# apschera2023uzk/MWR_fast_forward_operators_and_LBLs

Measured on AMD Instinct MI355X. Metric: TB evaluations/sec (profile x channel x angle), higher is better.
Workload: dtype f64

## Files before the change

### mwr_fast_forward_operators_and_lbls_amd/csrc/mwrt_kernels.hip.h

```cpp
#pragma once
#include <hip/hip_runtime.h>
#include <stdint.h>
#include "../../include/mwrt.h"
#include "mwrt_plan.h"

namespace mwrt {

constexpr double TAUMAX = 125.0;
constexpr double TRANS_MIN = 5.1664206328378610e-55;

struct O2Rec { double f, s300rf2, be, w300, y0, y1, g0, g1, dnu0, dnu1, pad[6]; };
struct H2ORec { double fl, s1, b2, w0, x, w0s, xs, sh, xh, shs, xhs, aair, aself, w2, pad[2]; };
struct ModelFlat : mwrt_model_desc {
  double o2_rf2[MWRT_MAX_O2_LINES];
  O2Rec o2r[MWRT_MAX_O2_LINES];
  H2ORec h2or[MWRT_MAX_H2O_LINES];
};
typedef const __attribute__((address_space(4))) ModelFlat* cmodel;
typedef const __attribute__((address_space(4))) double* cdoubles;

__device__ __forceinline__ int div_small(int n, int d, unsigned magic) {
  return d == 1 ? n : (int)__umulhi((unsigned)n, magic);
}

#ifndef MWRT_EXACT_DIV
#define MWRT_EXACT_DIV 0
#endif
#ifndef MWRT_ABLATE
#define MWRT_ABLATE 0
#endif
#ifndef MWRT_PHASE_CLOCK
#define MWRT_PHASE_CLOCK 0
#endif
#ifndef MWRT_NO_SETPRIO
#define MWRT_NO_SETPRIO 0
#endif
#if MWRT_NO_SETPRIO
#define MWRT_SETPRIO(n) do { } while (0)
#else
#define MWRT_SETPRIO(n) __builtin_amdgcn_s_setprio(n)
#endif
#if MWRT_PHASE_CLOCK
#define MWRT_STAMP(k) do { if (A.phase && lane == 0) A.phase[((int64_t)blockIdx.x * 4 + wave) * 10 + (k)] = (long long)wall_clock64(); } while (0)
#else
#define MWRT_STAMP(k) do { } while (0)
#endif

__device__ __forceinline__ double fdiv(double x, double d) {
#if MWRT_EXACT_DIV
  return x / d;
#else
  double r = __builtin_amdgcn_rcp(d);
  double e = __builtin_fma(-d, r, 1.0);
  r = __builtin_fma(r, e, r);
  e = __builtin_fma(-d, r, 1.0);
  r = __builtin_fma(r, e, r);
  return x * r;
#endif
}

#define MWRT_FMA_SC(p, r, c) asm("v_fma_f64 %0, %1, %2, %3" : "=v"(p) : "v"(p), "v"(r), "s"(c))
__device__ __forceinline__ double fexp(double x) {
#if MWRT_EXACT_DIV
  return exp(x);
#else
  const double k = __builtin_rint(x * 1.4426950408889634074);
  double r = __builtin_fma(k, -6.93147180369123816490e-01, x);
  r = __builtin_fma(k, -1.90821492927058770002e-10, r);
  double p = 2.5100569275813683e-08;
  MWRT_FMA_SC(p, r, 2.762032742826824e-07);
  MWRT_FMA_SC(p, r, 2.75572680728901e-06);
  MWRT_FMA_SC(p, r, 2.4801520792572694e-05);
  MWRT_FMA_SC(p, r, 0.00019841269863303223);
  MWRT_FMA_SC(p, r, 0.0013888888917538296);
  MWRT_FMA_SC(p, r, 0.008333333333330011);
  MWRT_FMA_SC(p, r, 0.04166666666662348);
  MWRT_FMA_SC(p, r, 0.16666666666666669);
  MWRT_FMA_SC(p, r, 0.5000000000000001);
  p = __builtin_fma(p, r, 1.0);
  p = __builtin_fma(p, r, 1.0);
  return __builtin_amdgcn_ldexp(p, (int)k);
#endif
}

__device__ __forceinline__ double two_atanh_tail(double z) {
  double p = 0.14616878919029822;
  MWRT_FMA_SC(p, z, 0.15331686868638428);
  MWRT_FMA_SC(p, z, 0.1818289017031397);
  MWRT_FMA_SC(p, z, 0.22222211120449298);
  MWRT_FMA_SC(p, z, 0.2857142862606338);
  MWRT_FMA_SC(p, z, 0.3999999999989931);
  MWRT_FMA_SC(p, z, 0.666666666666667);
  return p;
}

__device__ __forceinline__ double flog(double x) {
#if MWRT_EXACT_DIV
  return log(x);
#else
  int e = __builtin_amdgcn_frexp_exp(x);
  double m = __builtin_amdgcn_frexp_mant(x);
  const bool lo = m < 0.70710678118654752440;
  m = lo ? m + m : m;
  e = lo ? e - 1 : e;
  const double num = m - 1.0, den = m + 1.0;
  double r = __builtin_amdgcn_rcp(den);
  r = __builtin_fma(r, __builtin_fma(-den, r, 1.0), r);
  r = __builtin_fma(r, __builtin_fma(-den, r, 1.0), r);
  const double s = num * r;
  const double z = s * s;
  const double p = two_atanh_tail(z);
  const double ed = (double)e;
  const double lm = __builtin_fma(s * z, p, s + s);
  return __builtin_fma(ed, 6.93147180369123816490e-01, __builtin_fma(ed, 1.90821492927058770002e-10, lm));
#endif
}

constexpr double EXP_SMALL_X = 0.125;
__device__ __forceinline__ double fexp_small(double x) {
  double p = 2.756514908613403e-06;
  MWRT_FMA_SC(p, x, 2.4810200365624755e-05);
  MWRT_FMA_SC(p, x, 0.00019841269076602318);
  MWRT_FMA_SC(p, x, 0.001388888804772704);
  MWRT_FMA_SC(p, x, 0.008333333333357229);
  MWRT_FMA_SC(p, x, 0.04166666666692954);
  MWRT_FMA_SC(p, x, 0.16666666666666666);
  MWRT_FMA_SC(p, x, 0.4999999999999999);
  p = __builtin_fma(p, x, 1.0);
  return __builtin_fma(p, x, 1.0);
}

__device__ __forceinline__ double ftanh_half_small(double x) {
  const double u = x * x;
  double p = 4.257889640378761e-05;
  MWRT_FMA_SC(p, u, -0.0004216256671577941);
  MWRT_FMA_SC(p, u, 0.004166666662552237);
  MWRT_FMA_SC(p, u, -0.04166666666666466);
  p = __builtin_fma(p, u, 0.5);
  return p * x;
}

constexpr double EXP_TINY_X = 0.015625;
__device__ __forceinline__ double fexp_tiny(double x) {
  double p = 1.3888888888888889e-03;
  MWRT_FMA_SC(p, x, 8.3333333333333332e-03);
  MWRT_FMA_SC(p, x, 4.1666666666666664e-02);
  MWRT_FMA_SC(p, x, 1.6666666666666666e-01);
  p = __builtin_fma(p, x, 0.5);
  p = __builtin_fma(p, x, 1.0);
  return __builtin_fma(p, x, 1.0);
}
__device__ __forceinline__ double ftanh_half_tiny(double x) {
  const double u = x * x;
  double p = -4.2162698412698413e-04;
  MWRT_FMA_SC(p, u, 4.1666666666666666e-03);
  MWRT_FMA_SC(p, u, -4.1666666666666664e-02);
  p = __builtin_fma(p, u, 0.5);
  return p * x;
}

typedef unsigned long long wmask;
__device__ __forceinline__ bool wave_all(bool p) { return __builtin_amdgcn_ballot_w64(!p) == 0ull; }
__device__ __forceinline__ bool wave_any(bool p) { return __builtin_amdgcn_ballot_w64(p) != 0ull; }
__device__ __forceinline__ wmask wballot(bool p) { return __builtin_amdgcn_ballot_w64(p); }
template <class... B>
__device__ __forceinline__ bool wave_all_of(B... b) { return (wballot(b) & ...) == wballot(true); }

__device__ __forceinline__ float row16_max(float m) {
  m = fmaxf(m, __int_as_float(__builtin_amdgcn_update_dpp(0, __float_as_int(m), 0x128, 0xf, 0xf, false)));
  m = fmaxf(m, __int_as_float(__builtin_amdgcn_update_dpp(0, __float_as_int(m), 0x124, 0xf, 0xf, false)));
  m = fmaxf(m, __int_as_float(__builtin_amdgcn_update_dpp(0, __float_as_int(m), 0x122, 0xf, 0xf, false)));
  m = fmaxf(m, __int_as_float(__builtin_amdgcn_update_dpp(0, __float_as_int(m), 0x121, 0xf, 0xf, false)));
  return m;
}
constexpr int K2_SORT_MIN_SEGLEN = 16;

constexpr double PLANCK_SMALL_X = 0.03125;
__device__ __forceinline__ double planck_b(double x, double inv_x) {
  if (wave_all_of(x <= PLANCK_SMALL_X, x > 0.0)) {
    const double u = x * x;
    double g = 3.3068783068783071e-05;
    MWRT_FMA_SC(g, u, -1.3888888888888889e-03);
    MWRT_FMA_SC(g, u, 8.3333333333333329e-02);
    g = __builtin_fma(g, u, 1.0);
    g = __builtin_fma(x, -0.5, g);
    return g * inv_x;
  }
  return fdiv(1.0, fexp(x) - 1.0);
}

__device__ __forceinline__ double fdiv1(double x, double d) {
#if MWRT_EXACT_DIV
  return x / d;
#else
  double r = __builtin_amdgcn_rcp(d);
  r = __builtin_fma(r, __builtin_fma(-d, r, 1.0), r);
  return x * r;
#endif
}

#define LDS_RELOAD_FENCE() asm volatile("" ::: "memory")
#define KEEP_BRANCH() asm volatile("")

typedef const __attribute__((address_space(4))) LineMasks* cmasks;
__device__ __forceinline__ LineMasks load_masks(const LineMasks* table, int chunk) {
  const cmasks q = (cmasks)table + chunk;
  LineMasks lm;
  lm.o2_far = q->o2_far; lm.h2o_far = q->h2o_far; lm.h2o_none = q->h2o_none; lm.h2o_res = q->h2o_res; lm.h2o_sd = q->h2o_sd;
  lm.h2o_sdfar = q->h2o_sdfar; lm.h2o_sdint = q->h2o_sdint;
  lm.h2o_vfar = q->h2o_vfar; lm.o2_vfar = q->o2_vfar; lm.vf_u0 = q->vf_u0; lm.vf_h = q->vf_h; lm.vf_invh = q->vf_invh;
  return lm;
}

struct cplx { double re, im; };
__device__ __forceinline__ cplx cmul(cplx a, cplx b) { return {a.re * b.re - a.im * b.im, a.re * b.im + a.im * b.re}; }
__device__ __forceinline__ cplx cadd(cplx a, double r) { return {a.re + r, a.im}; }
__device__ __forceinline__ cplx crecip(cplx b) {
  const double d = __builtin_fma(b.re, b.re, b.im * b.im);
#if MWRT_EXACT_DIV
  const double r = 1.0 / d;
#else
  double r = __builtin_amdgcn_rcp(d);
  r = __builtin_fma(r, __builtin_fma(-d, r, 1.0), r);
  r = __builtin_fma(r, __builtin_fma(-d, r, 1.0), r);
#endif
  return {b.re * r, -b.im * r};
}
__device__ __forceinline__ cplx cdiv(cplx a, cplx b) { return cmul(a, crecip(b)); }
__device__ __forceinline__ double fsqrt(double x) {
#if MWRT_EXACT_DIV
  return sqrt(x);
#else
  const double y = __builtin_amdgcn_rsq(x);
  double g = x * y;
  const double h = 0.5 * y;
  return __builtin_fma(__builtin_fma(-g, g, x), h, g);
#endif
}
__device__ __forceinline__ cplx csqrt_principal(cplx z) {
  const double r = fsqrt(__builtin_fma(z.re, z.re, z.im * z.im));
  const bool pos = z.re >= 0.0;
  const double a = fsqrt(0.5 * (r + fabs(z.re)));
  const double q = fdiv1(pos ? z.im : fabs(z.im), a + a);
  return pos ? cplx{a, q} : cplx{q, copysign(a, z.im)};
}

__device__ __forceinline__ cplx dcerror_upper(double x, double y) {
  const double a0 = 122.607931777104326, a1 = 214.382388694706425, a2 = 181.928533092181549,
               a3 = 93.155580458138441, a4 = 30.180142196210589, a5 = 5.912626209773153,
               a6 = 0.564189583562615;
  const double b0 = 122.607931773875350, b1 = 352.730625110963558, b2 = 457.334478783897737,
               b3 = 348.703917719495792, b4 = 170.354001821091472, b5 = 53.992906912940207,
               b6 = 10.479857114260399;
  const cplx zh = {fabs(y), -x};
  const double r = zh.re + zh.re;
  const double ms = -__builtin_fma(zh.re, zh.re, zh.im * zh.im);
  auto step = [&](double c, double b1, double b2) -> double { return __builtin_fma(r, b1, __builtin_fma(ms, b2, c)); };
  double n2 = a6, n1 = __builtin_fma(r, a6, a5), nt;
  nt = step(a4, n1, n2); n2 = n1; n1 = nt;
  nt = step(a3, n1, n2); n2 = n1; n1 = nt;
  nt = step(a2, n1, n2); n2 = n1; n1 = nt;
  nt = step(a1, n1, n2); n2 = n1; n1 = nt;
  const cplx as = {__builtin_fma(zh.re, n1, __builtin_fma(ms, n2, a0)), zh.im * n1};
  double d2 = 1.0, d1 = r + b6, dt;
  dt = __builtin_fma(r, d1, ms + b5); d2 = d1; d1 = dt;
  dt = step(b4, d1, d2); d2 = d1; d1 = dt;
  dt = step(b3, d1, d2); d2 = d1; d1 = dt;
  dt = step(b2, d1, d2); d2 = d1; d1 = dt;
  dt = step(b1, d1, d2); d2 = d1; d1 = dt;
  const cplx bs = {__builtin_fma(zh.re, d1, __builtin_fma(ms, d2, b0)), zh.im * d1};
  return cdiv(as, bs);
}

__device__ __forceinline__ double block_sum(double v, double* scratch , int tid, int nthreads) {
#pragma unroll
  for (int o = WAVE / 2; o > 0; o >>= 1) v += __shfl_xor(v, o, WAVE);
  __syncthreads();
  if ((tid & (WAVE - 1)) == 0) scratch[tid / WAVE] = v;
  __syncthreads();
  double s = 0.0;
  for (int w = 0; w < nthreads / WAVE; ++w) s += scratch[w];
  return s;
}

struct LevelState {
  double t;
  double p;
  double rho;
  double pdry;
};

__device__ __forceinline__ double goff_gratch_e(double tk, double rh) {
  const double LN10 = 2.302585092994045684;
  const double INV_LN10 = 0.434294481903251828;
  double y = 373.16 / tk;
  double es = -7.90298 * (y - 1.0) + 5.02808 * (flog(y) * INV_LN10)
            - 1.3816e-07 * (fexp(LN10 * (11.344 * (1.0 - (1.0 / y)))) - 1.0)
            + 0.0081328 * (fexp(LN10 * (-3.49149 * (y - 1.0))) - 1.0) + 3.0057148979490314 ;
  return rh * fexp(LN10 * es);
}

__device__ __forceinline__ LevelState level_state(double p_hpa, double tk, double e) {
  const double rvap = (0.01 * 8.314510) / 18.01528;
  double v = 300.0 / tk;
  double ekpa = e / 10.0;
  double pdrykpa = p_hpa / 10.0 - ekpa;
  LevelState s;
  s.t = 300.0 / v;
  s.p = (pdrykpa + ekpa) * 10.0;
  s.rho = ekpa * 10.0 / (rvap * s.t);
  s.pdry = pdrykpa * 10.0;
  return s;
}

struct H2OLine {
  double c1;
  double w0, wsq;
  double sw;
  double sbase;
  double s;
  double base;
};

__device__ __forceinline__ H2OLine h2o_line(cmodel M, int k, double pda, double pvap, double ti, double tiln,
                                            double ti2, bool shifted) {
  H2OLine q;
  const auto& R = M->h2or[k];
  const double fl = R.fl;
// ... 725 lines not shown
    const double fl = M->x_fl[k];
    const double wc = M->x_w[k] * p * fexp(M->x_x[k] * tiln);
    const double bd = sq * fl;
    const double w = 0.5346 * wc + fsqrt(__builtin_fma(0.2166 * wc, wc, 0.6931 * (bd * bd)));
    const double wsq = w * w;
    const double sw = (M->x_s1[k] * fexp(M->x_b[k] * (1.0 - ti))) * fdiv(w, fl * fl);
    LDS_RELOAD_FENCE();
#pragma unroll
    for (int j = 0; j < NFC; ++j) {
      const double f = sfq[2 * j];
      const double d1 = f - fl, d2 = f + fl;
      const double D1 = __builtin_fma(d1, d1, wsq), D2 = __builtin_fma(d2, d2, wsq);
      const double den12 = D1 * D2;
      double r = __builtin_amdgcn_rcp(den12);
      r = __builtin_fma(r, __builtin_fma(-den12, r, 1.0), r);
      sum[j] = __builtin_fma((D1 + D2) * r, sw, sum[j]);
    }
  }
  const double pref = ((M->x_coef * numden) * qvinv) * fexp(2.5 * tiln);
#pragma unroll
  for (int j = 0; j < NFC; ++j) adry[j] = __builtin_fma(pref * sfq[2 * j + 1], sum[j], adry[j]);
}

#ifdef MWRT_HOST_TU
constexpr double EARTH_RADIUS_KM = 6370.949;
__global__ void __launch_bounds__(1024)
k_ray_paths(const double* __restrict__ z, const double* __restrict__ p, const double* __restrict__ t,
            const double* __restrict__ rh, int nlev, const double* __restrict__ elev_deg, int nang,
            double* __restrict__ amf, uint8_t* __restrict__ duct) {
  __shared__ double seam[16][3];
  const int64_t prof = blockIdx.x;
  const int tid = threadIdx.x, lane = tid & (WAVE - 1), wave = tid / WAVE;
  const bool active = tid < nlev;
  const int64_t off = prof * nlev + (active ? tid : 0);
  const double qnan = __builtin_nan("");
  const double z0 = z[prof * nlev];
  const double zi = z[off] - z0;
  const double pi = p[off], ti = t[off], rhi = rh[off];
  const bool bad_prof = __syncthreads_or(active && (isnan(zi) || isnan(pi) || isnan(ti) || isnan(rhi)));
  const double ni = thayer_refindex(pi, ti, goff_gratch_e(ti, rhi));
  if (lane == WAVE - 1) seam[wave][0] = ni;
  __syncthreads();
  double nprev = __shfl_up(ni, 1, WAVE);
  double zprev = __shfl_up(zi, 1, WAVE);
  if (lane == 0 && wave > 0) { nprev = seam[wave - 1][0]; zprev = z[off - 1] - z0; }
  const double n0 = thayer_refindex(p[prof * nlev], t[prof * nlev], goff_gratch_e(t[prof * nlev], rh[prof * nlev]));
  const double rs = EARTH_RADIUS_KM + 0.0 + z0;
  const double r = EARTH_RADIUS_KM + zi + z0;
  const double rl = EARTH_RADIUS_KM + zprev + z0;
  const double dz = zi - zprev;
  double refbar;
  if (ni == nprev || ni == 1.0 || nprev == 1.0) refbar = (ni + nprev) * 0.5;
  else refbar = 1.0 + (nprev - ni) / (log((nprev - 1.0) / (ni - 1.0)));
  for (int a = 0; a < nang; ++a) {
    double* out = amf + (prof * nang + a) * nlev;
    const double angle = elev_deg[a];
    if (bad_prof || isnan(angle)) {
      if (active) out[tid] = tid == 0 ? 0.0 : qnan;
      continue;
    }
    if ((angle >= 89.0 && angle <= 91.0) || (angle >= -91.0 && angle <= -89.0)) {
      if (active) out[tid] = (tid > 0 && dz != 0.0) ? 1.0 : 0.0;
      continue;
    }
    const double theta0 = angle * (M_PI / 180.0);
    const double costh0 = cos(theta0), sina = sin(theta0 * 0.5);
    const double a0 = 2.0 * (sina * sina);
    const double argdth = zi / rs - ((n0 - ni) * costh0 / ni);
    const double argth = 0.5 * (a0 + argdth) / r;
    const bool trapped_here = active && tid > 0 && !(argth > 0.0);
    double theta = theta0, dtheta = 0.0;
    if (tid > 0 && argth > 0.0) {
      const double sint = sqrt(r * argth);
      theta = 2.0 * asin(sint);
      if ((theta - 2.0 * theta0) <= 0.0) {
        const double dendth = 2.0 * (sint + sina) * cos((theta + theta0) * 0.25);
        const double sind4 = (0.5 * argdth - zi * argth) / dendth;
        dtheta = 4.0 * asin(sind4);
        theta = theta0 + dtheta;
      } else {
        dtheta = theta - theta0;
      }
    }
    const double tanth = tan(theta);
    __syncthreads();
    if (lane == WAVE - 1) { seam[wave][1] = tanth; seam[wave][2] = dtheta; }
    const bool trapped = __syncthreads_or(trapped_here);
    double tanthl = __shfl_up(tanth, 1, WAVE);
    double dthl = __shfl_up(dtheta, 1, WAVE);
    if (lane == 0 && wave > 0) { tanthl = seam[wave - 1][1]; dthl = seam[wave - 1][2]; }
    double f = 0.0;
    if (tid > 0) {
      const double cthbar = ((1.0 / tanth) + (1.0 / tanthl)) * 0.5;
      const double dtau = cthbar * (nprev - ni) / refbar;
      const double dphi = (dtheta - dthl) + dtau;
      const double sh = sin(dphi * 0.5);
      double dsi = sqrt(dz * dz + 4.0 * r * rl * (sh * sh));
      if (dtau != 0.0) {
        const double dtaua = fabs(dtau);
        dsi = dsi * (dtaua / (2.0 * sin(dtaua * 0.5)));
      }
      f = (dz != 0.0) ? dsi / dz : 0.0;
    }
    if (active) out[tid] = trapped ? (tid == 0 ? 0.0 : qnan) : f;
    if (trapped && tid == 0) duct[prof] = 1;
  }
}

#endif

struct FusedArgs {
  const ModelFlat* Ms[MAX_MULTI];
  int64_t nprof_in;
  const double* z; const double* p; const double* t; const double* rh;
  const double* frq;
  const double* airmass;
  double* tb;
  uint8_t* valid;
  double* tbatm; double* tmr; double* tauwet; double* taudry;
  double* taulay;
  int nlev, nf, nang;
  int write_valid;
  LaunchGeom g;
  const double* denliq; const double* denice;
  const double* amf;
  const uint8_t* duct;
  double* tauliq; double* tauice;
  const double* awet_in; const double* adry_in;
  const LineMasks* masks[MAX_MULTI];
  const double* o3n;
#if MWRT_PHASE_CLOCK
  long long* phase;
#endif
};

__device__ __forceinline__ void blank_outputs(const FusedArgs& A, int64_t prof, int jbase, int nfc, int tid, int nthreads) {
  const double qnan = __builtin_nan("");
  const int nang = A.nang, nlev = A.nlev;
  for (int it = tid; it < nfc * nang; it += nthreads) {
    const int j = it / nang, a = it % nang;
    const int64_t o = (prof * nang + a) * A.nf + jbase + j;
    A.tb[o] = qnan;
    if (A.tbatm) A.tbatm[o] = qnan;
    if (A.tmr) A.tmr[o] = qnan;
    if (A.tauwet) A.tauwet[o] = qnan;
    if (A.taudry) A.taudry[o] = qnan;
    if (A.tauliq) A.tauliq[o] = qnan;
    if (A.tauice) A.tauice[o] = qnan;
  }
  if (A.taulay) for (int it = tid; it < nfc * nlev; it += nthreads)
    A.taulay[(prof * A.nf + jbase + it / nlev) * nlev + it % nlev] = qnan;
}

#ifndef MWRT_MIN_WAVES
#define MWRT_MIN_WAVES 1
#endif
template <int NFC, int NFK, int MAXT, bool OPT = false, bool EXTRAS = false, bool ALPHA = false>
__global__ void __launch_bounds__(MAXT, (MAXT <= 256 ? (EXTRAS ? MWRT_MIN_WAVES : (ALPHA ? 4 : 3)) : 1))
k_tb_fused(const FusedArgs A) {
  constexpr int NPASS = (NFC + NFK - 1) / NFK;
  static_assert(NPASS <= 2, "LaunchGeom carries the split of two passes");
  extern __shared__ __attribute__((aligned(16))) double lds[];
  const int tid = threadIdx.x;
  const int lane = tid & (WAVE - 1);
  const int wave = tid / WAVE;
  const int nthreads = blockDim.x;
  const int nwaves = nthreads / WAVE;
  const int64_t prof = blockIdx.x;
  const int mi = (int)(prof / A.nprof_in);
  const int64_t pin = prof - mi * A.nprof_in;
  const int jbase = blockIdx.y * NFC;
  const int nfc = min(NFC, A.nf - jbase);
  const int nlev = A.nlev, nang = A.nang, ld = A.g.ldrow;
  const cmodel M = (cmodel)A.Ms[mi];
  const cdoubles cfrq = (cdoubles)A.frq;
  const cdoubles cam = (cdoubles)A.airmass;

  double* tau = lds;
  double* bof = tau + (size_t)NFK * ld;
  double* part = bof + (size_t)NFK * ld;
  double* scratch = part + (size_t)A.g.npart;
  double* edge = scratch + 16;
  constexpr int GRP = 16;
  const int ngrp = nthreads / GRP;
  float* gmax = (float*)(edge + (size_t)nwaves * 2 * NFC);
  int* wcnt = (int*)(gmax + (size_t)NFK * ngrp);
  int* perm = wcnt + nwaves;
  __shared__ int s_flag;
  __shared__ double sfq[5 * NFC + 2];

  MWRT_STAMP(0);
#if MWRT_PHASE_CLOCK
  if (A.phase && lane == 0) {
    A.phase[((int64_t)blockIdx.x * 4 + wave) * 10 + 8] = (long long)__builtin_amdgcn_s_getreg((31 << 11) | 4);
    A.phase[((int64_t)blockIdx.x * 4 + wave) * 10 + 9] = (long long)__builtin_amdgcn_s_getreg((31 << 11) | 20);
  }
#endif
  if (tid == 0) s_flag = 0;
  if (tid < NFC) {
    const double f = cfrq[jbase + min(tid, nfc - 1)];
    sfq[2 * tid] = f; sfq[2 * tid + 1] = f * f;
    double fdep = 1.0;
    if (M->n2_fdep) { const double q = f * (1.0 / 450.0); fdep = 0.5 + fdiv(0.5, 1.0 + q * q); }
    sfq[2 * NFC + 2 + tid] = fdep;
    sfq[3 * NFC + 2 + tid] = fdiv(1.0, f);
    sfq[4 * NFC + 2 + tid] = fdiv(1.0, fexp(fdiv(f * (1e9 * M->planck_h / M->boltzmann_k), M->t_cosmic)) - 1.0);
  }
  if (tid == WAVE - 1) {
    double lo = cfrq[jbase], hi = lo;
    for (int j = 1; j < nfc; ++j) { const double f = cfrq[jbase + j]; lo = fmin(lo, f); hi = fmax(hi, f); }
    sfq[2 * NFC] = lo; sfq[2 * NFC + 1] = hi;
  }
  __syncthreads();

  const bool active = tid < nlev;
  const bool wave_live = wave * WAVE < nlev;
  const int64_t off = pin * nlev + (active ? tid : 0);
  const double zi = A.z[off], ti = A.t[off];
  const double pi = ALPHA ? 0.0 : A.p[off], rhi = ALPHA ? 0.0 : A.rh[off];
  if (active && (isnan(zi) || isnan(pi) || isnan(ti) || isnan(rhi))) atomicOr(&s_flag, 1);
  double awet[NFC], adry[NFC];
  if constexpr (ALPHA) {
    bool bad = false;
    if (wave_live) {
#pragma unroll
      for (int j = 0; j < NFC; ++j) {
        const int64_t o = (pin * A.nf + jbase + min(j, nfc - 1)) * nlev + (active ? tid : 0);
        awet[j] = A.awet_in[o];
        adry[j] = A.adry_in[o];
        bad = bad || isnan(awet[j]) || isnan(adry[j]);
      }
    } else {
#pragma unroll
      for (int j = 0; j < NFC; ++j) { awet[j] = 0.0; adry[j] = 0.0; }
    }
    if (active && bad) atomicOr(&s_flag, 1);
  }
  double denl = 0.0, deni = 0.0, o3n = 0.0;
  if constexpr (OPT) {
    if (A.denliq) denl = A.denliq[off];
    if (A.denice) deni = A.denice[off];
    if (A.o3n) o3n = A.o3n[off];
    if (active && (isnan(denl) || isnan(deni) || isnan(o3n))) atomicOr(&s_flag, 1);
  }
  __syncthreads();
  if (s_flag) {
    blank_outputs(A, prof, jbase, nfc, tid, nthreads);
    if (tid == 0) A.valid[prof] = 0;
    return;
  }

  if constexpr (!ALPHA) {
    const double e = goff_gratch_e(ti, rhi);
    const LevelState L = level_state(pi, ti, e);
    const LineMasks lm = load_masks(A.masks[mi], blockIdx.y);
    MWRT_STAMP(1);
    MWRT_SETPRIO(3);
    h2o_absorb<NFC>(M, L, sfq, lm, awet);
    MWRT_STAMP(2);
    MWRT_SETPRIO(2);
    dry_absorb<NFC>(M, L, sfq, lm, adry);
    MWRT_SETPRIO(1);
    MWRT_STAMP(3);
    if constexpr (OPT) {
      if (A.o3n) x_absorb<NFC>(M, ti, pi, o3n, sfq, adry);
    }
  }
  if (lane == WAVE - 1) {
#pragma unroll
    for (int j = 0; j < NFC; ++j) { edge[wave * 2 * NFC + j] = awet[j]; edge[wave * 2 * NFC + NFC + j] = adry[j]; }
  }
  __syncthreads();
  double tw[EXTRAS ? NFC : 1], td[NFC];
  bool neg = false;
  {
    const double z0 = A.z[pin * nlev];
    const double dz = (active && tid > 0) ? ((zi - z0) - (A.z[off - 1] - z0)) : 0.0;
    const bool seam = (lane == 0) && (wave > 0);
    const bool has_prev = active && tid > 0;
    if (!wave_live) {
#pragma unroll
      for (int j = 0; j < NFC; ++j) { td[j] = 0.0; if constexpr (EXTRAS) tw[j] = 0.0; }
    } else
#pragma unroll
    for (int j = 0; j < NFC; ++j) {
#pragma clang fp contract(off)
      double pw = __shfl_up(awet[j], 1, WAVE);
      double pd = __shfl_up(adry[j], 1, WAVE);
      if (seam) { pw = edge[(wave - 1) * 2 * NFC + j]; pd = edge[(wave - 1) * 2 * NFC + NFC + j]; }
      const double lw = layer_value(awet[j], pw, neg, has_prev), ld_ = layer_value(adry[j], pd, neg, has_prev);
      const double twj = has_prev ? lw * dz : 0.0;
      const double tdj = has_prev ? ld_ * dz : 0.0;
      if constexpr (EXTRAS) { tw[j] = twj; td[j] = tdj; }
      else td[j] = twj + tdj;
    }
  }
  constexpr bool CLOUD_ROWS = OPT && EXTRAS;
  double tl[CLOUD_ROWS ? NFC : 1], tci[CLOUD_ROWS ? NFC : 1];
  if constexpr (OPT) {
#pragma unroll
    for (int j = 0; j < (CLOUD_ROWS ? NFC : 1); ++j) { tl[j] = 0.0; tci[j] = 0.0; }
    const bool cloud_here = active && (denl > 0.0 || deni > 0.0);
    if ((A.denliq || A.denice) && __syncthreads_or(cloud_here)) {
      auto row = [&](int j) -> double* { return (j < NFK ? tau + (size_t)j * ld : bof + (size_t)(j - NFK) * ld); };
      {
        const CloudLevel cl = cloud_level(M, ti);
        if (active) {
#pragma unroll
          for (int j = 0; j < NFC; ++j) row(j)[tid] = (denl > 0.0) ? liquid_abs(cl, sfq[2 * j], denl) : 0.0;
        }
      }
      __syncthreads();
      const bool has_below = active && tid > 0;
      const double deni_prev = (has_below && A.denice) ? A.denice[off - 1] : 0.0;
      const double z0 = A.z[pin * nlev];
      const double dz = has_below ? ((zi - z0) - (A.z[off - 1] - z0)) : 0.0;
#pragma unroll
      for (int j = 0; j < NFC; ++j) {
        const double f = sfq[2 * j];
        const double al = active ? row(j)[tid] : 0.0;
        const double pl = has_below ? row(j)[tid - 1] : 0.0;
        const double ai = (deni > 0.0) ? CLOUD_KICE * f * deni : 0.0;
        const double pc = (deni_prev > 0.0) ? CLOUD_KICE * f * deni_prev : 0.0;
        const double ll = layer_value<false>(al, pl, neg, has_below), li = layer_value<false>(ai, pc, neg, has_below);
        const double tlj = has_below ? ll * dz : 0.0;
        const double tij = has_below ? li * dz : 0.0;
        if constexpr (CLOUD_ROWS) { tl[j] = tlj; tci[j] = tij; }
        else td[j] = (td[j] + tij) + tlj;
      }
      __syncthreads();
    }
  }
  MWRT_STAMP(4);
  if (neg) atomicOr(&s_flag, 2);
  __syncthreads();
  if (s_flag) {
    blank_outputs(A, prof, jbase, nfc, tid, nthreads);
    if (tid == 0) A.valid[prof] = 2;
    return;
  }
  const double hk = 1e9 * M->planck_h / M->boltzmann_k;
  const double inv_hk = 1e-9 * M->boltzmann_k / M->planck_h;
  bool want_tau = false;
  if constexpr (EXTRAS) {
    if (A.taulay && active) {
#pragma unroll
      for (int j = 0; j < NFC; ++j)
        if (j < nfc) {
          double tz = tw[j] + td[j];
          if constexpr (CLOUD_ROWS) tz = (tz + tci[j]) + tl[j];
          A.taulay[(prof * A.nf + jbase + j) * nlev + tid] = tz;
        }
    }
    want_tau = (A.tauwet != nullptr) || (A.taudry != nullptr) || (A.tauliq != nullptr) || (A.tauice != nullptr);
  }

#pragma unroll
  for (int h = 0; h < NPASS; ++h) {
    const int nfk = min(NFK, nfc - h * NFK);
    if (nfk <= 0) break;
    if (h > 0) MWRT_SETPRIO(0);
    if (h > 0) __syncthreads();
    const int nseg = A.g.nseg[h], seglen = A.g.seglen[h];
    const int npairs = nfk * nang;
    const int items = (MWRT_ABLATE & 8) ? 0 : npairs * nseg;
    const bool sorted = !(OPT && A.amf) && items <= nthreads && seglen >= K2_SORT_MIN_SEGLEN;
    if (wave_live) {
      const double hkt = fdiv(hk, ti);
      const double kth = ti * inv_hk;
#pragma unroll
      for (int jj = 0; jj < NFK; ++jj) {
        const int j = h * NFK + jj;
        if (j < NFC) {
          double tz = td[j];
          if constexpr (EXTRAS) tz = tw[j] + td[j];
          if constexpr (CLOUD_ROWS) tz = (tz + tci[j]) + tl[j];
          const double bz = planck_b(sfq[2 * j] * hkt, sfq[3 * NFC + 2 + j] * kth);
          if (active) { tau[jj * ld + tid] = tz; bof[jj * ld + tid] = bz; }
          if (sorted) {
            const float m = row16_max(active ? (float)tz * 1.0000005f : 0.0f);
            if ((lane & (GRP - 1)) == 0) gmax[jj * ngrp + tid / GRP] = m;
          }
        }
      }
    }
    double swet[EXTRAS ? NFK : 1], sdry[EXTRAS ? NFK : 1], sliq[EXTRAS ? NFK : 1], sice[EXTRAS ? NFK : 1];
    const bool rays = OPT && A.amf != nullptr;
    if constexpr (EXTRAS) {
      if (want_tau && !rays) {
#pragma unroll
        for (int jj = 0; jj < NFK; ++jj) {
          constexpr int JL = NFC - 1;
          const int j = min(h * NFK + jj, JL);
          swet[jj] = block_sum(tw[j], scratch, tid, nthreads);
          sdry[jj] = block_sum(td[j], scratch, tid, nthreads);
          if constexpr (OPT) {
            sliq[jj] = block_sum(tl[j], scratch, tid, nthreads);
            sice[jj] = block_sum(tci[j], scratch, tid, nthreads);
          } else {
            sliq[jj] = 0.0; sice[jj] = 0.0;
          }
        }
      }
    }
    if constexpr (EXTRAS && OPT) {
      if (want_tau && rays) {
        const int npairs_r = nfk * nang;
        for (int sp = 0; sp < 4; ++sp) {
          double* outp = sp == 0 ? A.tauwet : sp == 1 ? A.taudry : sp == 2 ? A.tauliq : A.tauice;
          __syncthreads();
          if (active) {
#pragma unroll
            for (int jj = 0; jj < NFK; ++jj) {
              const int j = h * NFK + jj;
              if (j < NFC) tau[jj * ld + tid] = sp == 0 ? tw[j] : sp == 1 ? td[j] : sp == 2 ? tl[j] : tci[j];
            }
          }
          __syncthreads();
          if (outp) for (int pr = tid; pr < npairs_r; pr += nthreads) {
            const int jj = pr / nang, a = pr - jj * nang;
            const double* fr = A.amf + (pin * nang + a) * nlev;
            double acc = 0.0;
            for (int i = 1; i < nlev; ++i) acc += tau[jj * ld + i] * fr[i];
            outp[(prof * nang + a) * A.nf + jbase + h * NFK + jj] = acc;
          }
        }
        __syncthreads();
        if (active) {
#pragma unroll
          for (int jj = 0; jj < NFK; ++jj) {
            const int j = h * NFK + jj;
            if (j < NFC) tau[jj * ld + tid] = ((tw[j] + td[j]) + tci[j]) + tl[j];
          }
        }
      }
    }
    __syncthreads();

    int nthin_all = 0;
    if (sorted) {
      const bool mine = tid < items;
      const int it = mine ? tid : 0;
      const int pr = div_small(it, nseg, A.g.magic_nseg[h]), seg = it - pr * nseg;
      const int jj = div_small(pr, nang, A.g.magic_nang), a = pr - jj * nang;
      const int lo = 1 + seg * seglen, hi = min(lo + seglen, nlev);
      float gm = 0.0f;
      for (int g = lo / GRP; g <= (hi - 1) / GRP; ++g) gm = fmaxf(gm, gmax[jj * ngrp + g]);
      const bool thin = mine && !((double)gm * cam[a] > EXP_SMALL_X);
      const unsigned long long bal = __ballot(thin);
      const int rank = __popcll(bal & ((1ull << lane) - 1ull));
      if (lane == 0) wcnt[wave] = __popcll(bal);
      __syncthreads();
      int before = 0, nthin = 0;
      for (int w = 0; w < nwaves; ++w) { const int c = wcnt[w]; nthin += c; if (w < wave) before += c; }
      if (mine) perm[thin ? before + rank : nthin + tid - (before + rank)] = (a << 11) | (jj << 7) | seg;
      nthin_all = nthin;
      __syncthreads();
    }
    for (int it0 = tid; it0 < items; it0 += nthreads) {
      int seg, jj, a;
      if (sorted) {
        const int key = perm[it0];
        seg = key & 127; jj = (key >> 7) & 15; a = key >> 11;
      } else {
        const int pr = div_small(it0, nseg, A.g.magic_nseg[h]);
        seg = it0 - pr * nseg; jj = div_small(pr, nang, A.g.magic_nang); a = pr - jj * nang;
      }
      const int it = (jj * nang + a) * nseg + seg;
      const double am = cam[a];
      const int lo = 1 + seg * seglen;
      const int hi = min(lo + seglen, nlev);
      const double* tj = tau + jj * ld;
      const double* bj = bof + jj * ld;
      const double* fr = nullptr;
      if constexpr (OPT) fr = A.amf ? A.amf + (pin * nang + a) * nlev : nullptr;
      double T = 1.0, B = 0.0;
      double bprev = (lo < nlev) ? bj[lo - 1] : 0.0;
      if (!sorted) {
        for (int i = lo; i < hi; ++i) {
          const double tl = tj[i] * ((OPT && fr) ? fr[i] : am);
          const double E = wave_all(fabs(tl) <= EXP_SMALL_X) ? fexp_small(-tl) : fexp(-tl);
          const double bi = bj[i];
          const double lay = fdiv1(__builtin_fma(bi, E, bprev), 1.0 + E);
          B = __builtin_fma(lay * T, 1.0 - E, B);
          T *= E;
          bprev = bi;
        }
      } else if (wave_all(it0 < nthin_all)) {
        auto step = [&](double tz, double bi) {
          const double tl = tz * am;
          const double E = fexp_small(-tl);
          const double th = ftanh_half_small(tl);
          B = __builtin_fma(__builtin_fma(bi, E, bprev) * T, th, B);
          T *= E;
          bprev = bi;
        };
        int i = lo;
        double t0 = (i < hi) ? tj[i] : 0.0, b0 = (i < hi) ? bj[i] : 0.0;
        for (; i + 1 < hi; i += 2) {
          const double t1 = tj[i + 1], b1 = bj[i + 1];
          const double t2 = tj[i + 2], b2 = bj[i + 2];
          step(t0, b0); step(t1, b1);
          t0 = t2; b0 = b2;
        }
        if (i < hi) step(t0, b0);
      } else {
        auto step = [&](double tz, double bi) {
          const double tl = tz * am;
          const double E = fexp(-tl);
          const double lay = fdiv1(__builtin_fma(bi, E, bprev), 1.0 + E);
          B = __builtin_fma(lay * T, 1.0 - E, B);
          T *= E;
          bprev = bi;
        };
        int i = lo;
        double t0 = (i < hi) ? tj[i] : 0.0, b0 = (i < hi) ? bj[i] : 0.0;
        for (; i + 1 < hi; i += 2) {
          const double t1 = tj[i + 1], b1 = bj[i + 1];
          const double t2 = tj[i + 2], b2 = bj[i + 2];
          step(t0, b0); step(t1, b1);
          t0 = t2; b0 = b2;
        }
        if (i < hi) step(t0, b0);
      }
      part[2 * it + 0] = B; part[2 * it + 1] = T;
    }
    MWRT_STAMP(5 + h);
    __syncthreads();
    for (int pr = tid; pr < npairs; pr += nthreads) {
      const int jj = div_small(pr, nang, A.g.magic_nang);
      const int a = pr - jj * nang;
      const int j = h * NFK + jj;
      double B = 0.0, T = 1.0;
      for (int sg = 0; sg < nseg; ++sg) {
        const double* q = part + 2 * (pr * nseg + sg);
        B = __builtin_fma(T, q[0], B);
        T *= q[1];
      }
      const double hvk = cfrq[jbase + j] * hk;
      double boftotl, boftmr;
      if (T > TRANS_MIN) {
        const double ex = T;
        const double bbg = sfq[4 * NFC + 2 + j];
        boftotl = __builtin_fma(bbg, ex, B);
        boftmr = EXTRAS ? fdiv(B, 1.0 - ex) : 0.0;
      } else {
        boftotl = B; boftmr = B;
      }
      const int64_t o = (prof * nang + a) * A.nf + jbase + j;
      A.tb[o] = fdiv(hvk, flog(1.0 + fdiv(1.0, boftotl)));
      if constexpr (EXTRAS) {
        if (A.tbatm) A.tbatm[o] = fdiv(hvk, flog(1.0 + fdiv(1.0, B)));
        if (A.tmr) A.tmr[o] = fdiv(hvk, flog(1.0 + fdiv(1.0, boftmr)));
        if (want_tau && !rays) {
          const double am = cam[a];
          double sw = 0.0, sd = 0.0, sl = 0.0, si = 0.0;
#pragma unroll
          for (int q2 = 0; q2 < NFK; ++q2) if (q2 == jj) { sw = swet[q2]; sd = sdry[q2]; sl = sliq[q2]; si = sice[q2]; }
          if (A.tauwet) A.tauwet[o] = sw * am;
          if (A.taudry) A.taudry[o] = sd * am;
          if (A.tauliq) A.tauliq[o] = sl * am;
          if (A.tauice) A.tauice[o] = si * am;
        }
      }
    }
  }
  if constexpr (OPT) {
    if (A.duct && A.duct[pin]) { if (tid == 0) A.valid[prof] = 3; return; }
  }
  if (A.write_valid && tid == 0) A.valid[prof] = 1;
  MWRT_STAMP(7);
}

struct TauOut {
  const double* z;
  double* tau;
  uint8_t* valid;
  int fpitch;
};

__device__ __forceinline__ double lane_below(double v) {
  const long long b = __builtin_bit_cast(long long, v);
  const int lo = (int)b, hi = (int)(b >> 32);
  const int plo = __builtin_amdgcn_update_dpp(lo, lo, 0x138, 0xf, 0xf, false);
  const int phi = __builtin_amdgcn_update_dpp(hi, hi, 0x138, 0xf, 0xf, false);
  return __builtin_bit_cast(double, ((long long)phi << 32) | (unsigned)plo);
}

template <class RowOk>
__device__ __forceinline__ void store_tau_chunk(const double (&tz)[TAU_NFC], double* tau_prof , int64_t fpitch,
                                                int lev0, int lane, RowOk row_ok) {
  if (row_ok(lev0 + lane, lane)) {
    double2* row = (double2*)(tau_prof + (int64_t)(lev0 + lane) * fpitch);
#pragma unroll
    for (int j = 0; j < TAU_NFC; j += 2) row[j / 2] = double2{tz[j], tz[j + 1]};
  }
}

template <int NFC, class ModelPtr>
__device__ __forceinline__ void fill_chunk_table(double* sfq, ModelPtr M, cdoubles cfrq, int jbase, int nfc, int lane) {
  __builtin_amdgcn_wave_barrier();
  asm volatile("" ::: "memory");
  if (lane < NFC) {
    const double f = cfrq[jbase + min(lane, nfc - 1)];
    sfq[2 * lane] = f; sfq[2 * lane + 1] = f * f;
    double fdep = 1.0;
    if (M->n2_fdep) { const double q = f * (1.0 / 450.0); fdep = 0.5 + fdiv(0.5, 1.0 + q * q); }
    sfq[2 * NFC + 2 + lane] = fdep;
  }
  if (lane == WAVE - 1) {
    double lo = cfrq[jbase], hi = lo;
    for (int j = 1; j < nfc; ++j) { const double f = cfrq[jbase + j]; lo = fmin(lo, f); hi = fmax(hi, f); }
    sfq[2 * NFC] = lo; sfq[2 * NFC + 1] = hi;
  }
  __builtin_amdgcn_wave_barrier();
  asm volatile("" ::: "memory");
}

__device__ __forceinline__ void blank_tau(const TauOut& T, int64_t prof, int nlev, int c0, int nch, int tid, int nthreads) {
  const double qnan = __builtin_nan("");
  const int w = nch * TAU_NFC;
  for (int it = tid; it < nlev * w; it += nthreads) {
    const int l = it / w, k = it - l * w;
    T.tau[(prof * nlev + l) * (int64_t)T.fpitch + c0 * TAU_NFC + k] = qnan;
  }
}

struct AbsorbArgs {
  const ModelFlat* M;
  const double* p; const double* t; const double* rh;
  const double* frq;
  double* awet; double* adry;
  int nlev, nf;
  TauOut T;
  const LineMasks* masks;
};

template <int NFC, int MAXT, bool TAU = false>
__global__ void __launch_bounds__(MAXT)
k_absorb(const AbsorbArgs A) {
  static_assert(!TAU || NFC == TAU_NFC, "tau rows are written in 16-frequency pieces");
  const int tid = threadIdx.x;
  const int lane = tid & (WAVE - 1), wave = tid / WAVE;
  const int64_t prof = blockIdx.x;
  const int jbase = blockIdx.y * NFC;
  const int nfc = min(NFC, A.nf - jbase);
  const cmodel M = (cmodel)A.M;
  const cdoubles cfrq = (cdoubles)A.frq;
  __shared__ double sfq_w[MAXT / WAVE][3 * NFC + 2];
  double* sfq = sfq_w[wave];
  fill_chunk_table<NFC>(sfq, M, cfrq, jbase, nfc, lane);
  const int lev = TAU ? wave * (WAVE - 1) + lane : tid;
  const bool active = lev < A.nlev;
  const int64_t off = prof * A.nlev + (active ? lev : 0);
  const double pi = A.p[off], ti = A.t[off], rhi = A.rh[off];
  double zi = 0.0;
  if constexpr (TAU) {
    zi = A.T.z[off];
    if (__syncthreads_or(active && (isnan(zi) || isnan(pi) || isnan(ti) || isnan(rhi)))) {
      blank_tau(A.T, prof, A.nlev, blockIdx.y, 1, tid, blockDim.x);
      if (tid == 0) A.T.valid[prof] = 0;
      return;
    }
  }
  double awet[NFC], adry[NFC];
  const double e = goff_gratch_e(ti, rhi);
  const LevelState L = level_state(pi, ti, e);
  const LineMasks lm = load_masks(A.masks, blockIdx.y);
  h2o_absorb<NFC>(M, L, sfq, lm, awet);
  dry_absorb<NFC>(M, L, sfq, lm, adry);
  if constexpr (!TAU) {
    if (active) {
#pragma unroll
      for (int j = 0; j < NFC; ++j) {
        if (j < nfc) {
          const int64_t o = (prof * A.nf + jbase + j) * A.nlev + tid;
// ... 463 lines not shown
```

### mwr_fast_forward_operators_and_lbls_amd/csrc/mwrt_plan.cpp

```cpp
#include "mwrt_plan.h"

#include <algorithm>
#include <cmath>
#include <cstdlib>
#include <cstring>

namespace mwrt {

namespace {

int plan_k2_pass(int nlev, int npairs, int threads) {
  const int layers = nlev - 1;
  int best = 1; long best_cost = -1;
  for (int ns = 1; ns <= 64 && ns <= (layers > 0 ? layers : 1); ++ns) {
    const int sl = (layers + ns - 1) / ns;
    const long rounds = ((long)npairs * ns + threads - 1) / threads;
    const long cost = rounds * (sl * 8L + 4) + ns;
    if (best_cost < 0 || cost < best_cost) { best_cost = cost; best = ns; }
  }
  return best;
}

int rows0_of(int nfc, int nf) { return std::min(NFK, std::min(nfc, nf)); }
int rows1_of(int nfc, int nf) { return std::max(0, std::min(nfc, nf) - NFK); }

void set_pass(LaunchGeom* g, int h, int nlev, int ns) {
  g->nseg[h] = ns < 1 ? 1 : ns;
  g->seglen[h] = (nlev - 1 + g->nseg[h] - 1) / g->nseg[h];
  if (g->seglen[h] < 1) g->seglen[h] = 1;
}

void set_split(LaunchGeom* g, int nlev, int nfc, int nf, int nang, int ns0, int ns1) {
  set_pass(g, 0, nlev, ns0);
  set_pass(g, 1, nlev, ns1);
  g->npart = 2 * nang * std::max(rows0_of(nfc, nf) * g->nseg[0], rows1_of(nfc, nf) * g->nseg[1]);
  g->magic_nseg[0] = magic_of(g->nseg[0]);
  g->magic_nseg[1] = magic_of(g->nseg[1]);
  g->magic_nang = magic_of(nang);
}

LaunchGeom plan_k2(int nlev, int nfc, int nf, int nang, int threads) {
  LaunchGeom g;
  const int rows1 = rows1_of(nfc, nf);
  set_split(&g, nlev, nfc, nf, nang, plan_k2_pass(nlev, rows0_of(nfc, nf) * nang, threads),
            rows1 > 0 ? plan_k2_pass(nlev, rows1 * nang, threads) : 1);
  int ld = nlev + 1;
  if ((ld & 1) == 0) ld += 1;
  g.ldrow = ld;
  return g;
}

size_t fused_lds_bytes(int nfc, const LaunchGeom& g, int threads) {
  const size_t sort_doubles = ((size_t)NFK * (threads / 16) + (threads / WAVE) + threads + 1) / 2;
  return sizeof(double) * ((size_t)2 * NFK * g.ldrow + (size_t)g.npart + 16 +
                           (size_t)(threads / WAVE) * 2 * nfc + sort_doubles);
}

double sd_halfwidth_bound(const mwrt_model_desc& t, int k) {
  return t.h2o_w0[k] * 1100.0 * std::pow(2.0, std::max(t.h2o_x[k], 0.0)) +
         t.h2o_w0s[k] * 150.0 * std::pow(2.0, std::max(t.h2o_xs[k], 0.0));
}

template <int NNODES>
void window_nodes(const double* frq, int b, int e, int nchunks, double* fnode, double* blk_base) {
  const int per = nchunks * WIN_NFC;
  const double flo = frq[b], fhi = frq[e];
  long double x[NNODES], bw[NNODES];
  for (int m = 0; m < NNODES; ++m)
    fnode[m] = (double)(0.5L * (flo + fhi) + 0.5L * (fhi - flo) * cosl(M_PIl * (2 * m + 1) / (2.0L * NNODES)));
  for (int m = 0; m < NNODES; ++m) x[m] = fnode[m];
  for (int m = 0; m < NNODES; ++m) {
    long double prod = 1.0L;
    for (int k = 0; k < NNODES; ++k) if (k != m) prod *= (x[m] - x[k]);
    bw[m] = 1.0L / prod;
  }
  for (int r = 0; r < per; ++r) {
    const long double f = frq[std::min(b + r, e)];
    const int cidx = r / WIN_NFC, j = r % WIN_NFC;
    double* blk = blk_base + (size_t)cidx * NNODES * WIN_NFC;
    int hit = -1;
    for (int m = 0; m < NNODES; ++m) if (f == x[m]) hit = m;
    if (hit >= 0) { blk[hit * WIN_NFC + j] = 1.0; continue; }
    long double q[NNODES], sum = 0.0L;
    for (int m = 0; m < NNODES; ++m) { q[m] = bw[m] / (f - x[m]); sum += q[m]; }
    for (int m = 0; m < NNODES; ++m) blk[m * WIN_NFC + j] = (double)(q[m] / sum);
  }
}

void window_far_sets(const mwrt_model_desc& t, double flo, double fhi, WinDesc* d) {
  const double half = 0.5 * (fhi - flo);
  const double mo = std::max(WIN_MARGIN_GHZ, 1.6 * half), mh = std::max(WIN_H2O_MARGIN_GHZ, 11.8 * half);
  d->o2_far = 0; d->h2o_far_both = 0; d->h2o_far_res = 0;
  for (int k = 0; k < t.n_o2; ++k) {
    const double c = t.o2_f[k];
    if (c < flo - mo || c > fhi + mo) d->o2_far |= 1ull << k;
  }
  for (int k = 0; k < t.n_h2o; ++k) {
    const double c = t.h2o_fl[k];
    if (!(c < flo - mh || c > fhi + mh)) continue;
    if (t.h2o_w2[k] > 0.0 && !(10.0 * sd_halfwidth_bound(t, k) < std::min(std::fabs(c - flo), std::fabs(c - fhi)) - 1.0)) continue;
    const double g = WIN_CUTOFF_GUARD_GHZ;
    const bool d1_in = std::fabs(flo - c) < 750.0 - g && std::fabs(fhi - c) < 750.0 - g;
    const bool d2_in = fhi + c < 750.0 - g;
    const bool d2_out = flo + c >= 750.0 + g;
    if (d1_in && d2_in) d->h2o_far_both |= 1u << k;
    else if (d1_in && d2_out) d->h2o_far_res |= 1u << k;
  }
}

size_t up256(size_t x) { return (x + 255) & ~(size_t)255; }

}

unsigned magic_of(int d) { return d <= 1 ? 0u : (unsigned)((((uint64_t)1 << 32) + (uint64_t)d - 1) / (uint64_t)d); }

bool plan_fused(int lds_max, int nfc, int nlev, int nf, int nang, LaunchGeom* g, size_t* lds, int threads) {
  if (threads <= 0) threads = lanes_for(nlev);
  *g = plan_k2(nlev, nfc, nf, nang, threads);
  *lds = fused_lds_bytes(nfc, *g, threads);
  while (*lds > (size_t)lds_max && (g->nseg[0] > 1 || g->nseg[1] > 1)) {
    set_split(g, nlev, nfc, nf, nang, (g->nseg[0] + 1) / 2, (g->nseg[1] + 1) / 2);
    *lds = fused_lds_bytes(nfc, *g, threads);
  }
  return *lds <= (size_t)lds_max;
}

int pick_nfc(int nf) {
  if (nf % 14 == 0 || nf <= 14) return (nf <= 8) ? 8 : 14;
  return 16;
}

int pick_nfc_fused(int chunk_width, int lds_max, int nlev, int nf, int nang) {
  int nfc = chunk_width ? chunk_width : pick_nfc(nf);
  LaunchGeom g; size_t lds;
  if (!plan_fused(lds_max, nfc, nlev, nf, nang, &g, &lds)) nfc = 8;
  return nfc;
}

bool any_nan(const double* x, int n) {
  for (int i = 0; i < n; ++i) if (std::isnan(x[i])) return true;
  return false;
}

bool all_nan(const double* x, int n) {
  for (int i = 0; i < n; ++i) if (!std::isnan(x[i])) return false;
  return true;
}

bool airmass_of(const double* elev, int nang, std::vector<double>* am) {
  am->resize(nang);
  for (int a = 0; a < nang; ++a) {
    if (std::isnan(elev[a])) { (*am)[a] = std::nan(""); continue; }
    if (!(elev[a] > 0.0 && elev[a] < 180.0)) return false;
    (*am)[a] = 1.0 / std::sin(elev[a] * M_PI / 180.0);
  }
  return true;
}

int rte_tau_angles(int rem) { return rem <= 8 ? rem : (rem == 10 ? 10 : (rem == 9 ? 5 : 8)); }

int tau_pitch_of(int nf) { return ((nf + TAU_NFC - 1) / TAU_NFC) * TAU_NFC; }

size_t absorb_win_lds_bytes(int threads) {
  const int maxt = threads <= 256 ? 256 : 512;
  return sizeof(double) * ((size_t)(WIN_NODES + WIN_NODES_H) * threads + (3 * WIN_NFC + 2) * (1 + maxt / WAVE) +
                           (3 * WIN_NODES_H + 2)) + 64;
}

bool windows_eligible(const double* frq, int nf) {
  if (nf < WIN_CHUNKS * WIN_NFC) return false;
  for (int j = 1; j < nf; ++j) if (!(frq[j] > frq[j - 1])) return false;
  const int per = WIN_CHUNKS * WIN_NFC;
  for (int b = 0; b < nf; b += per) {
    const int e = std::min(nf, b + per) - 1;
    if (e == b) return false;
    if (frq[e] - frq[b] > WIN_MAX_SPAN_GHZ) return false;
  }
  return true;
}

AbsorbRoute absorption_route(int mode, int lds_max, const double* frq, int nf, int threads) {
  const bool ok = windows_eligible(frq, nf) && threads <= 512 && absorb_win_lds_bytes(threads) <= (size_t)lds_max;
  if (mode == 2 && !ok) return AbsorbRoute::refused;
  return ok && mode != 1 ? AbsorbRoute::windowed : AbsorbRoute::every_line;
}

void chunk_masks(const mwrt_model_desc& t, const double* frq, int nf, int nfc, std::vector<LineMasks>* out) {
  const int nchunks = (nf + nfc - 1) / nfc;
  out->assign(nchunks, LineMasks{});
  for (int ch = 0; ch < nchunks; ++ch) {
    const int j0 = ch * nfc, j1 = std::min(nf, j0 + nfc);
    LineMasks& lm = (*out)[ch];
    double ulo = 1e300, uhi = 0.0;
    for (int j = j0; j < j1; ++j) { ulo = std::min(ulo, frq[j] * frq[j]); uhi = std::max(uhi, frq[j] * frq[j]); }
    lm.vf_u0 = 0.5 * (ulo + uhi);
    lm.vf_h = std::max(0.5 * (uhi - ulo), 1.0);
    lm.vf_invh = 1.0 / lm.vf_h;
    auto very_far = [&](double c) {
      const double cl = std::max(c - 2.0, 0.0), ch = c + 2.0;
      const double plo = cl * cl - 100.0, phi = ch * ch;
      const double dist = (lm.vf_u0 < plo) ? plo - lm.vf_u0 : ((lm.vf_u0 > phi) ? lm.vf_u0 - phi : 0.0);
// ... 138 lines not shown
```

### mwr_fast_forward_operators_and_lbls_amd/csrc/mwrt_plan.h

```cpp
#pragma once
#include <stddef.h>
#include <stdint.h>
#include <vector>
#include "../../include/mwrt.h"

namespace mwrt {

constexpr int WAVE = 64;

struct LaunchGeom {
  int nseg[2];
  int seglen[2];
  int npart;
  int ldrow;
  unsigned magic_nseg[2];
  unsigned magic_nang;
};

constexpr double FAR_MIN_GHZ = 0.2;
constexpr double FAR_SHIFT_GHZ = 0.05;
constexpr double FAR_H2O_GHZ = 5.0;

struct LineMasks {
  unsigned long long o2_far;
  unsigned h2o_far;
  unsigned h2o_none;
  unsigned h2o_res;
  unsigned h2o_sd;
  unsigned h2o_sdfar;
  unsigned h2o_sdint;
  unsigned h2o_vfar;
  unsigned long long o2_vfar;
  double vf_u0, vf_h, vf_invh;
};

constexpr double VF_RATIO_MAX = 0.016;
constexpr int VF_MIN_FREQS = 7;
constexpr int VF_MIN_LINES = 4;

constexpr int SD_NODES = 9, SD_TARGETS = 7;
constexpr int sd_node_slot(int n) { return n < 8 ? 2 * n : 15; }

constexpr int MAX_MULTI = 8;

constexpr int NFK = 8;

constexpr int TAU_NFC = 16;
constexpr int tau_threads(int nlev) { return ((nlev - 1 + (WAVE - 2)) / (WAVE - 1)) * WAVE; }
constexpr int lanes_for(int nlev) { return ((nlev + WAVE - 1) / WAVE) * WAVE; }

constexpr int WIN_NODES = 16;
constexpr int WIN_NODES_H = 8;
constexpr int WIN_CHUNKS = 8;
constexpr int WIN_CHUNKS_MAX = 16;
constexpr int WIN_NFC = 16;

struct WinDesc {
  double fnode[WIN_NODES];
  double fnode_h[WIN_NODES_H];
  double flo, fhi;
  unsigned long long o2_far;
  unsigned h2o_far_both, h2o_far_res;
  int first_chunk, nchunks;
  int pad0, pad1;
};

constexpr int RTE_THREADS = 256;

constexpr double WIN_MARGIN_GHZ = 4.0;
constexpr double WIN_H2O_MARGIN_GHZ = 30.0;
constexpr double WIN_MAX_SPAN_GHZ = 6.0;
constexpr double WIN_CUTOFF_GUARD_GHZ = 5.0;

unsigned magic_of(int d);

bool plan_fused(int lds_max, int nfc, int nlev, int nf, int nang, LaunchGeom* g, size_t* lds, int threads = 0);
int pick_nfc(int nf);
int pick_nfc_fused(int chunk_width, int lds_max, int nlev, int nf, int nang);

bool any_nan(const double* x, int n);
bool all_nan(const double* x, int n);
bool airmass_of(const double* elev, int nang, std::vector<double>* am);
int rte_tau_angles(int rem);
int tau_pitch_of(int nf);

size_t absorb_win_lds_bytes(int threads);
bool windows_eligible(const double* frq, int nf);
enum class AbsorbRoute { every_line, windowed, refused  };
AbsorbRoute absorption_route(int mode, int lds_max, const double* frq, int nf, int threads);

void chunk_masks(const mwrt_model_desc& t, const double* frq, int nf, int nfc, std::vector<LineMasks>* out);

struct WindowSet {
  std::vector<WinDesc> wins;
  std::vector<double> lag, lag_h;
  std::vector<double> lag_sd;
};
void build_windows(const mwrt_model_desc& t, const double* frq, int nf, WindowSet* ws);

struct WindowLayout { size_t off_lag, off_lagh, off_lagsd, total; };
WindowLayout window_layout(int nwin, int nf);
void pack_windows(const WindowSet& ws, int nf, std::vector<char>* blob);

struct RowArray { double* p; size_t per; };
void blank_rows(const uint8_t* valid, int64_t nrows, bool unless_one, const RowArray* arrays, int narrays);

}
```

Measured before the change: 966.0 million.

## Software-pipeline RTE segment loop with padded LDS rows and VGPR-pinned constants

Adds a shared rte_segment helper that walks each segment's tau and Planck values from LDS in steps of four. It prefetches the next loads ahead of each step and drops per-iteration bounds checks. To let the loop run past the last level without guarding, the row stride (ldrow) is padded to cover nseg*seglen, and the pad region is zeroed. The first polynomial coefficient of exp and tanh is also pinned in a VGPR so it is not rematerialized each iteration. The unsorted path uses the new loop when no per-level airmass is given. The costs are a larger LDS footprint, which can reduce occupancy, and the extra zeroing stores.

```diff
diff --git a/mwr_fast_forward_operators_and_lbls_amd/csrc/mwrt_kernels.hip.h b/mwr_fast_forward_operators_and_lbls_amd/csrc/mwrt_kernels.hip.h
--- a/mwr_fast_forward_operators_and_lbls_amd/csrc/mwrt_kernels.hip.h
+++ b/mwr_fast_forward_operators_and_lbls_amd/csrc/mwrt_kernels.hip.h
@@ -60,14 +60,19 @@
 }
 
 #define MWRT_FMA_SC(p, r, c) asm("v_fma_f64 %0, %1, %2, %3" : "=v"(p) : "v"(p), "v"(r), "s"(c))
-__device__ __forceinline__ double fexp(double x) {
+__device__ __forceinline__ double loop_invariant_vgpr(double c) {
+  asm volatile("" : "+v"(c));
+  return c;
+}
+constexpr double FEXP_C0 = 2.5100569275813683e-08;
+__device__ __forceinline__ double fexp(double x, double c0 = FEXP_C0) {
 #if MWRT_EXACT_DIV
   return exp(x);
 #else
   const double k = __builtin_rint(x * 1.4426950408889634074);
   double r = __builtin_fma(k, -6.93147180369123816490e-01, x);
   r = __builtin_fma(k, -1.90821492927058770002e-10, r);
-  double p = 2.5100569275813683e-08;
+  double p = c0;
   MWRT_FMA_SC(p, r, 2.762032742826824e-07);
   MWRT_FMA_SC(p, r, 2.75572680728901e-06);
   MWRT_FMA_SC(p, r, 2.4801520792572694e-05);
@@ -117,8 +122,9 @@
 }
 
 constexpr double EXP_SMALL_X = 0.125;
-__device__ __forceinline__ double fexp_small(double x) {
-  double p = 2.756514908613403e-06;
+constexpr double FEXP_SMALL_C0 = 2.756514908613403e-06;
+__device__ __forceinline__ double fexp_small(double x, double c0 = FEXP_SMALL_C0) {
+  double p = c0;
   MWRT_FMA_SC(p, x, 2.4810200365624755e-05);
   MWRT_FMA_SC(p, x, 0.00019841269076602318);
   MWRT_FMA_SC(p, x, 0.001388888804772704);
@@ -130,9 +136,10 @@
   return __builtin_fma(p, x, 1.0);
 }
 
-__device__ __forceinline__ double ftanh_half_small(double x) {
+constexpr double FTANH_HALF_SMALL_C0 = 4.257889640378761e-05;
+__device__ __forceinline__ double ftanh_half_small(double x, double c0 = FTANH_HALF_SMALL_C0) {
   const double u = x * x;
-  double p = 4.257889640378761e-05;
+  double p = c0;
   MWRT_FMA_SC(p, u, -0.0004216256671577941);
   MWRT_FMA_SC(p, u, 0.004166666662552237);
   MWRT_FMA_SC(p, u, -0.04166666666666466);
@@ -173,7 +180,6 @@
   m = fmaxf(m, __int_as_float(__builtin_amdgcn_update_dpp(0, __float_as_int(m), 0x121, 0xf, 0xf, false)));
   return m;
 }
-constexpr int K2_SORT_MIN_SEGLEN = 16;
 
 constexpr double PLANCK_SMALL_X = 0.03125;
 __device__ __forceinline__ double planck_b(double x, double inv_x) {
@@ -1205,6 +1211,29 @@
     A.taulay[(prof * A.nf + jbase + it / nlev) * nlev + it % nlev] = qnan;
 }
 
+typedef const __attribute__((address_space(3))) double* ldoubles;
+template <class Step>
+__device__ __forceinline__ void rte_segment(const double* tau_seg, const double* bof_seg, int seglen, Step step) {
+  ldoubles tp = (ldoubles)tau_seg, bp = (ldoubles)bof_seg;
+  asm volatile("" : "+v"(tp), "+v"(bp));
+  double t0 = tp[0], t1 = tp[1], b0 = bp[0], b1 = bp[1];
+  for (int n = seglen >> 2; n > 0; --n) {
+    const double t2 = tp[2], t3 = tp[3];
+    step(t0, b0);
+    const double b2 = bp[2], b3 = bp[3];
+    step(t1, b1);
+    t0 = tp[4]; t1 = tp[5];
+    step(t2, b2);
+    b0 = bp[4]; b1 = bp[5];
+    step(t3, b3);
+    tp += 4; bp += 4;
+  }
+  const int rest = seglen & 3;
+  if (rest > 0) step(t0, b0);
+  if (rest > 1) step(t1, b1);
+  if (rest > 2) step(tp[2], bp[2]);
+}
+
 #ifndef MWRT_MIN_WAVES
 #define MWRT_MIN_WAVES 1
 #endif
@@ -1408,6 +1437,11 @@
     want_tau = (A.tauwet != nullptr) || (A.taudry != nullptr) || (A.tauliq != nullptr) || (A.tauice != nullptr);
   }
 
+  for (int k = nlev + tid; k < ld; k += nthreads) {
+#pragma unroll
+    for (int jj = 0; jj < NFK; ++jj) { tau[jj * ld + k] = 0.0; bof[jj * ld + k] = 0.0; }
+  }
+
 #pragma unroll
   for (int h = 0; h < NPASS; ++h) {
     const int nfk = min(NFK, nfc - h * NFK);
@@ -1529,7 +1563,17 @@
       if constexpr (OPT) fr = A.amf ? A.amf + (pin * nang + a) * nlev : nullptr;
       double T = 1.0, B = 0.0;
       double bprev = (lo < nlev) ? bj[lo - 1] : 0.0;
-      if (!sorted) {
+      if (!sorted && !(OPT && fr) && nseg * seglen < ld) {
+        const double cs = loop_invariant_vgpr(FEXP_SMALL_C0), ce = loop_invariant_vgpr(FEXP_C0);
+        rte_segment(tj + lo, bj + lo, seglen, [&](double tz, double bi) {
+          const double tl = tz * am;
+          const double E = wave_all(fabs(tl) <= EXP_SMALL_X) ? fexp_small(-tl, cs) : fexp(-tl, ce);
+          const double lay = fdiv1(__builtin_fma(bi, E, bprev), 1.0 + E);
+          B = __builtin_fma(lay * T, 1.0 - E, B);
+          T *= E;
+          bprev = bi;
+        });
+      } else if (!sorted) {
         for (int i = lo; i < hi; ++i) {
           const double tl = tj[i] * ((OPT && fr) ? fr[i] : am);
           const double E = wave_all(fabs(tl) <= EXP_SMALL_X) ? fexp_small(-tl) : fexp(-tl);
@@ -1540,41 +1584,25 @@
           bprev = bi;
         }
       } else if (wave_all(it0 < nthin_all)) {
-        auto step = [&](double tz, double bi) {
+        const double ce = loop_invariant_vgpr(FEXP_SMALL_C0), ct = loop_invariant_vgpr(FTANH_HALF_SMALL_C0);
+        rte_segment(tj + lo, bj + lo, seglen, [&](double tz, double bi) {
           const double tl = tz * am;
-          const double E = fexp_small(-tl);
-          const double th = ftanh_half_small(tl);
+          const double E = fexp_small(-tl, ce);
+          const double th = ftanh_half_small(tl, ct);
           B = __builtin_fma(__builtin_fma(bi, E, bprev) * T, th, B);
           T *= E;
           bprev = bi;
-        };
-        int i = lo;
-        double t0 = (i < hi) ? tj[i] : 0.0, b0 = (i < hi) ? bj[i] : 0.0;
-        for (; i + 1 < hi; i += 2) {
-          const double t1 = tj[i + 1], b1 = bj[i + 1];
-          const double t2 = tj[i + 2], b2 = bj[i + 2];
-          step(t0, b0); step(t1, b1);
-          t0 = t2; b0 = b2;
-        }
-        if (i < hi) step(t0, b0);
+        });
       } else {
-        auto step = [&](double tz, double bi) {
+        const double ce = loop_invariant_vgpr(FEXP_C0);
+        rte_segment(tj + lo, bj + lo, seglen, [&](double tz, double bi) {
           const double tl = tz * am;
-          const double E = fexp(-tl);
+          const double E = fexp(-tl, ce);
           const double lay = fdiv1(__builtin_fma(bi, E, bprev), 1.0 + E);
           B = __builtin_fma(lay * T, 1.0 - E, B);
           T *= E;
           bprev = bi;
-        };
-        int i = lo;
-        double t0 = (i < hi) ? tj[i] : 0.0, b0 = (i < hi) ? bj[i] : 0.0;
-        for (; i + 1 < hi; i += 2) {
-          const double t1 = tj[i + 1], b1 = bj[i + 1];
-          const double t2 = tj[i + 2], b2 = bj[i + 2];
-          step(t0, b0); step(t1, b1);
-          t0 = t2; b0 = b2;
-        }
-        if (i < hi) step(t0, b0);
+        });
       }
       part[2 * it + 0] = B; part[2 * it + 1] = T;
     }
diff --git a/mwr_fast_forward_operators_and_lbls_amd/csrc/mwrt_plan.cpp b/mwr_fast_forward_operators_and_lbls_amd/csrc/mwrt_plan.cpp
--- a/mwr_fast_forward_operators_and_lbls_amd/csrc/mwrt_plan.cpp
+++ b/mwr_fast_forward_operators_and_lbls_amd/csrc/mwrt_plan.cpp
@@ -37,6 +37,11 @@
   g->magic_nseg[0] = magic_of(g->nseg[0]);
   g->magic_nseg[1] = magic_of(g->nseg[1]);
   g->magic_nang = magic_of(nang);
+  int ld = nlev + 1;
+  for (int h = 0; h < 2; ++h)
+    if (g->seglen[h] >= K2_SORT_MIN_SEGLEN) ld = std::max(ld, g->nseg[h] * g->seglen[h] + 1);
+  if ((ld & 1) == 0) ld += 1;
+  g->ldrow = ld;
 }
 
 LaunchGeom plan_k2(int nlev, int nfc, int nf, int nang, int threads) {
@@ -44,9 +49,6 @@
   const int rows1 = rows1_of(nfc, nf);
   set_split(&g, nlev, nfc, nf, nang, plan_k2_pass(nlev, rows0_of(nfc, nf) * nang, threads),
             rows1 > 0 ? plan_k2_pass(nlev, rows1 * nang, threads) : 1);
-  int ld = nlev + 1;
-  if ((ld & 1) == 0) ld += 1;
-  g.ldrow = ld;
   return g;
 }
 
diff --git a/mwr_fast_forward_operators_and_lbls_amd/csrc/mwrt_plan.h b/mwr_fast_forward_operators_and_lbls_amd/csrc/mwrt_plan.h
--- a/mwr_fast_forward_operators_and_lbls_amd/csrc/mwrt_plan.h
+++ b/mwr_fast_forward_operators_and_lbls_amd/csrc/mwrt_plan.h
@@ -44,6 +44,7 @@
 constexpr int MAX_MULTI = 8;
 
 constexpr int NFK = 8;
+constexpr int K2_SORT_MIN_SEGLEN = 16;
 
 constexpr int TAU_NFC = 16;
 constexpr int tau_threads(int nlev) { return ((nlev - 1 + (WAVE - 2)) / (WAVE - 1)) * WAVE; }
```

New measurement: 990.3 million (median of 6 runs). 2.5% higher.
